# swesterfeld/audiowmark

Measured on AMD Instinct MI355X. Metric: audio seconds watermarked+decoded per wall-second (xRT), 44.1 kHz stereo, higher is better.
Workload: dtype f32; 1 GPU; 60 min stereo 44.1 kHz white noise per GPU resident in HBM, add+get incl. payload decode, payload 0123456789abcdef0011223344556677, strength 10; parallelism=1 GPU, patterns=108, payload_matches=104, ranks_seen=1

## Files before the change

### audiowmark_amd/csrc/hip/kernels.hip

```cpp
#include "kernels.hh"
#include "awm_fft.hip.h"
#include <cstdlib>
#include <algorithm>
#include <type_traits>
#include <atomic>

namespace awmk {

constexpr int NB = 81;
constexpr int MIN_BAND = 20;
constexpr int WAVES = 4;

typedef const int __attribute__ ((address_space (4))) *const_int_ptr;

__device__ __forceinline__ void
load_shared_tables (const DevTables& t, float2 *s_tw, float *s_win, float2 *s_twb)
{
  fft512_load_twiddles (t.tw512, s_tw);
  for (int i = threadIdx.x; i < 1024; i += blockDim.x)
    s_win[i] = t.window[i];
  if (s_twb)
    for (int i = threadIdx.x; i < NB; i += blockDim.x)
      s_twb[i] = t.tw1024[MIN_BAND + i];
}


__device__ __forceinline__ void
fetch_stereo (const float *pcm, long long idx, int avail, int lane, float (&l)[16], float (&r)[16])
{
  const float *p = pcm + idx * 2;
  if (avail >= 1024 && ((reinterpret_cast<uintptr_t> (p) & 15) == 0))
    {
      const float4 *p4 = reinterpret_cast<const float4 *> (p);
#pragma unroll
      for (int j = 0; j < 8; j++)
        {
          const float4 v = p4[lane + 64 * j];
          l[2 * j] = v.x; r[2 * j] = v.y; l[2 * j + 1] = v.z; r[2 * j + 1] = v.w;
        }
    }
  else if (avail >= 1024)
    {
      const float2 *p2 = reinterpret_cast<const float2 *> (p);
#pragma unroll
      for (int j = 0; j < 8; j++)
        {
          const float2 a = p2[2 * (lane + 64 * j)], b = p2[2 * (lane + 64 * j) + 1];
          l[2 * j] = a.x; r[2 * j] = a.y; l[2 * j + 1] = b.x; r[2 * j + 1] = b.y;
        }
    }
  else
    {
#pragma unroll
      for (int j = 0; j < 8; j++)
        {
          const int x = 2 * (lane + 64 * j);
          l[2 * j]     = x < avail     ? p[2 * x]     : 0.f;
          r[2 * j]     = x < avail     ? p[2 * x + 1] : 0.f;
          l[2 * j + 1] = x + 1 < avail ? p[2 * x + 2] : 0.f;
          r[2 * j + 1] = x + 1 < avail ? p[2 * x + 3] : 0.f;
        }
    }
}

__device__ __forceinline__ void
fetch_channel (const float *pcm, long long idx, int avail, int C, int ch, int lane, float (&v)[16])
{
  const float *p = pcm + idx * C + ch;
  if (C == 1 && avail >= 1024 && ((reinterpret_cast<uintptr_t> (p) & 7) == 0))
    {
      const float2 *p2 = reinterpret_cast<const float2 *> (p);
#pragma unroll
      for (int j = 0; j < 8; j++)
        {
          const float2 a = p2[lane + 64 * j];
          v[2 * j] = a.x; v[2 * j + 1] = a.y;
        }
    }
  else
    {
#pragma unroll
      for (int j = 0; j < 8; j++)
        {
          const int x = 2 * (lane + 64 * j);
          v[2 * j]     = x < avail     ? p[(long long) x * C]       : 0.f;
          v[2 * j + 1] = x + 1 < avail ? p[(long long) (x + 1) * C] : 0.f;
        }
    }
}

__device__ __forceinline__ void
window_pack (const float (&v)[16], const float *s_win, int lane, float2 (&z)[8])
{
  const float2 *w2 = reinterpret_cast<const float2 *> (s_win);
#pragma unroll
  for (int j = 0; j < 8; j++)
    {
      const float2 w = lds_ld (&w2[lane + 64 * j]);
      z[j] = make_float2 (__fmul_rn (v[2 * j], w.x), __fmul_rn (v[2 * j + 1], w.y));
    }
}

__global__ void __launch_bounds__ (64 * WAVES)
stft_full_kernel (DevTables t, const float *pcm, int C, long long start_index, long long hop, long long frame_count, float2 *out)
{
  __shared__ float2 s_tw[512];
  __shared__ float  s_win[1024];
  __shared__ float2 s_x[WAVES][XBUF_ELEMS];
  load_shared_tables (t, s_tw, s_win, nullptr);
  __syncthreads();

  const int lane = threadIdx.x & 63, wave = threadIdx.x >> 6;
  const long long item = (long long) blockIdx.x * WAVES + wave;
  if (item >= frame_count * C)
    return;
  const long long f = item / C;
  const int ch = int (item % C);
  float2 *xbuf = s_x[wave];

  float v[16];
  fetch_channel (pcm, start_index + f * hop, 1024, C, ch, lane, v);
  float2 z[8];
  window_pack (v, s_win, lane, z);
  fft512_forward (z, xbuf, s_tw, lane);
#pragma unroll
  for (int kc = 0; kc < 8; kc++)
    xbuf[kc * 64 + lane] = z[kc];
  wave_sync();
  float2 *o = out + item * 513;
  for (int k = lane; k <= 512; k += 64)
    {
      const float2 zk = xbuf[zpos (k & 511)], zm = xbuf[zpos ((512 - k) & 511)];
      o[k] = real_split (zk, zm, t.tw1024[k]);
    }
}

hipError_t
launch_stft_full (hipStream_t st, const DevTables& t, const float *pcm, int n_channels,
                  long long start_index, long long hop, long long frame_count, float2 *out)
{
  const long long items = frame_count * n_channels;
  if (items <= 0)
    return hipSuccess;
  const unsigned grid = unsigned ((items + WAVES - 1) / WAVES);
  hipLaunchKernelGGL (stft_full_kernel, dim3 (grid), dim3 (64 * WAVES), 0, st, t, pcm, n_channels, start_index, hop, frame_count, out);
  return hipGetLastError();
}


__device__ __forceinline__ int
zdpos (int k)
{
  const int kc = k >> 6;
  return (kc < 2 ? kc : kc - 4) * 64 + ((k >> 3) & 7) + 8 * (k & 7);
}


__device__ __forceinline__ void
frame_forward (float2 (&z)[8], float2 *xbuf, const float2 *s_tw, int lane)
{
  fft512_forward (z, xbuf, s_tw, lane);
  xbuf[0 * 64 + lane] = z[0];
  xbuf[1 * 64 + lane] = z[1];
  xbuf[6 * 64 + lane] = z[6];
  xbuf[7 * 64 + lane] = z[7];
  wave_sync();
}

__device__ __forceinline__ void
frame_forward2 (float2 (&za)[8], float2 (&zb)[8], float2 *xbuf, const float2 *s_tw, int lane)
{
  fft512_forward2 (za, zb, xbuf, s_tw, lane);
  lds_st (&xbuf[0 * 64 + lane], za[0]);
  lds_st (&xbuf[1 * 64 + lane], za[1]);
  lds_st (&xbuf[6 * 64 + lane], za[6]);
  lds_st (&xbuf[7 * 64 + lane], za[7]);
  lds_st (&xbuf[2 * 64 + lane], zb[0]);
  lds_st (&xbuf[3 * 64 + lane], zb[1]);
  lds_st (&xbuf[4 * 64 + lane], zb[6]);
  lds_st (&xbuf[5 * 64 + lane], zb[7]);
  wave_sync_pinned();
}

__device__ __forceinline__ int
zposb (int k)
{
  const int p = zpos (k);
  return p < 128 ? p + 128 : p - 128;
}

template<bool PINNED = false> __device__ __forceinline__ void
halfspec_store (float2 *zd, int k, float2 D, float2 O)
{
  const float2 lo = make_float2 (D.x - O.y, D.y + O.x), hi = make_float2 (D.x + O.y, O.x - D.y);
  if constexpr (PINNED)
    {
      lds_st (&zd[zdpos (k)], lo);
      lds_st (&zd[zdpos (512 - k)], hi);
    }
  else
    {
      zd[zdpos (k)] = lo;
      zd[zdpos (512 - k)] = hi;
    }
}

__device__ __forceinline__ void
frame_inverse (float2 (&z)[8], float2 *xbuf, float2 *zd, const float2 *s_tw, const float2 *s_tw3, int lane)
{
  wave_sync();
  const float2 zero = make_float2 (0.f, 0.f);
  z[0] = zd[0 * 64 + lane];
  z[1] = zd[1 * 64 + lane];
  z[2] = zero; z[3] = zero; z[4] = zero; z[5] = zero;
  z[6] = zd[2 * 64 + lane];
  z[7] = zd[3 * 64 + lane];
  wave_sync();
  fft512_inverse (z, xbuf, s_tw, s_tw3, lane);
}

__device__ __forceinline__ void
frame_inverse2 (float2 (&za)[8], float2 (&zb)[8], const float2 (&Da)[2], const float2 (&Oa)[2], const float2 (&Db)[2], const float2 (&Ob)[2],
                float2 *xbuf, float2 *zd, const float2 *s_tw, const float2 *s_tw3, int lane)
{
  const float2 zero = make_float2 (0.f, 0.f);
  wave_sync_pinned();
#pragma unroll
  for (int pass = 0; pass < 2; pass++)
    {
      const int k = MIN_BAND + lane + 64 * pass;
      if (k <= 100)
        halfspec_store<true> (zd, k, Da[pass], Oa[pass]);
    }
  wave_sync_pinned();
  za[0] = lds_ld (&zd[0 * 64 + lane]);
  za[1] = lds_ld (&zd[1 * 64 + lane]);
  za[2] = zero; za[3] = zero; za[4] = zero; za[5] = zero;
  za[6] = lds_ld (&zd[2 * 64 + lane]);
  za[7] = lds_ld (&zd[3 * 64 + lane]);
  wave_sync_pinned();
#pragma unroll
  for (int pass = 0; pass < 2; pass++)
    {
      const int k = MIN_BAND + lane + 64 * pass;
      if (k <= 100)
        halfspec_store<true> (zd, k, Db[pass], Ob[pass]);
    }
  wave_sync_pinned();
  zb[0] = lds_ld (&zd[0 * 64 + lane]);
  zb[1] = lds_ld (&zd[1 * 64 + lane]);
  zb[2] = zero; zb[3] = zero; zb[4] = zero; zb[5] = zero;
  zb[6] = lds_ld (&zd[2 * 64 + lane]);
  zb[7] = lds_ld (&zd[3 * 64 + lane]);
  wave_sync_pinned();
  fft512_inverse2 (za, zb, xbuf, s_tw, s_tw3, lane);
}

__device__ __forceinline__ void
frame_delta (float2 (&z)[8], const int8_t *mod_row, float nd_up, float nd_down,
             float2 *xbuf, float2 *zd, const float2 *s_tw, const float2 *s_tw3, const float2 *s_twb, int lane)
{
  frame_forward (z, xbuf, s_tw, lane);
#pragma unroll
  for (int pass = 0; pass < 2; pass++)
    {
      const int k = MIN_BAND + lane + 64 * pass;
      if (k <= 100)
        {
          const float2 w = s_twb[k - MIN_BAND];
          const float2 X = real_split (xbuf[zpos (k)], xbuf[zpos (512 - k)], w);
          const int mod = mod_row[k - MIN_BAND];
          float2 D = make_float2 (0.f, 0.f);
          if (mod)
            {
              const float abs2 = X.x * X.x + X.y * X.y;
              if (abs2 > 1e-14f)
                {
                  const float s = __builtin_amdgcn_exp2f (__builtin_amdgcn_logf (abs2) * (0.5f * (mod == 1 ? nd_up : nd_down))) - 1.0f;
                  D = make_float2 (X.x * s, X.y * s);
                }
            }
          halfspec_store (zd, k, D, cmulc (D, w));
        }
    }
  frame_inverse (z, xbuf, zd, s_tw, s_tw3, lane);
}

__device__ __forceinline__ void
frame_delta2 (float2 (&za)[8], float2 (&zb)[8], const int8_t *mod_row, float nd_up, float nd_down,
              float2 *xbuf, float2 *zd, const float2 *s_tw, const float2 *s_tw3, const float2 *s_twb, int lane)
{
  frame_forward2 (za, zb, xbuf, s_tw, lane);
  float2 Da[2], Db[2], Oa[2], Ob[2];
#pragma unroll
  for (int pass = 0; pass < 2; pass++)
    {
      const int k = MIN_BAND + lane + 64 * pass;
      Da[pass] = Db[pass] = Oa[pass] = Ob[pass] = make_float2 (0.f, 0.f);
      if (k <= 100)
        {
          const float2 w = s_twb[k - MIN_BAND];
          const float2 Xa = real_split (lds_ld (&xbuf[zpos (k)]), lds_ld (&xbuf[zpos (512 - k)]), w);
          const float2 Xb = real_split (lds_ld (&xbuf[zposb (k)]), lds_ld (&xbuf[zposb (512 - k)]), w);
          const int mod = mod_row[k - MIN_BAND];
          if (mod)
            {
              const float e = 0.5f * (mod == 1 ? nd_up : nd_down);
              const float abs2a = Xa.x * Xa.x + Xa.y * Xa.y, abs2b = Xb.x * Xb.x + Xb.y * Xb.y;
              if (abs2a > 1e-14f)
                {
                  const float s = __builtin_amdgcn_exp2f (__builtin_amdgcn_logf (abs2a) * e) - 1.0f;
                  Da[pass] = make_float2 (Xa.x * s, Xa.y * s);
                }
              if (abs2b > 1e-14f)
                {
                  const float s = __builtin_amdgcn_exp2f (__builtin_amdgcn_logf (abs2b) * e) - 1.0f;
                  Db[pass] = make_float2 (Xb.x * s, Xb.y * s);
                }
            }
          Oa[pass] = cmulc (Da[pass], w);
          Ob[pass] = cmulc (Db[pass], w);
        }
    }
  frame_inverse2 (za, zb, Da, Oa, Db, Ob, xbuf, zd, s_tw, s_tw3, lane);
}

__device__ __forceinline__ float
wave_max (float v)
{
#pragma unroll
  for (int off = 32; off > 0; off >>= 1)
    v = fmaxf (v, __shfl_xor (v, off));
  return v;
}

struct FramePlace
{
  bool own, own_prev;
  int b0, bound, pb0, pbound;
};

__device__ __forceinline__ FramePlace
frame_place (long long gs_m, int BS, long long first_block, bool own, bool own_prev)
{
  FramePlace fp;
  fp.own = own;
  fp.own_prev = own_prev;
  const long long b0 = gs_m >= 0 ? gs_m / BS : 0;
  const long long gs_p = gs_m - 1024;
  const long long pb0 = gs_p >= 0 ? gs_p / BS : 0;
  fp.b0 = int (b0 - first_block);
  fp.bound = int (std::min<long long> ((b0 + 1) * BS - gs_m, 2048));
  fp.pb0 = int (pb0 - first_block);
  fp.pbound = int (std::min<long long> ((pb0 + 1) * BS - gs_p, 2048));
  return fp;
}

template<int CV> __device__ __forceinline__ void
overlap_add_mix (float (&o)[CV][16], const float2 (&d)[CV][8], const float (&in)[CV][16], float (&head2)[CV][2], float (&tail_s1)[CV][2],
                 const float (&tail_in)[CV][2], float2 w1_head, float2 w2_head, float2 w1_tail, float2 w0_tail)
{
#pragma unroll
  for (int c = 0; c < CV; c++)
    {
      const float s1x = __fadd_rn (head2[c][0], __fmul_rn (d[c][0].x, w1_head.x));
      const float s1y = __fadd_rn (head2[c][1], __fmul_rn (d[c][0].y, w1_head.y));
      o[c][0] = __fadd_rn (s1x, in[c][0]);
      o[c][1] = __fadd_rn (s1y, in[c][1]);
      head2[c][0] = __fmul_rn (d[c][0].x, w2_head.x);
      head2[c][1] = __fmul_rn (d[c][0].y, w2_head.y);
#pragma unroll
      for (int j = 1; j < 7; j++)
        {
          o[c][2 * j]     = __fadd_rn (d[c][j].x, in[c][2 * j]);
          o[c][2 * j + 1] = __fadd_rn (d[c][j].y, in[c][2 * j + 1]);
        }
      o[c][14] = __fadd_rn (__fadd_rn (tail_s1[c][0], __fmul_rn (d[c][7].x, w0_tail.x)), tail_in[c][0]);
      o[c][15] = __fadd_rn (__fadd_rn (tail_s1[c][1], __fmul_rn (d[c][7].y, w0_tail.y)), tail_in[c][1]);
      tail_s1[c][0] = __fmul_rn (d[c][7].x, w1_tail.x);
      tail_s1[c][1] = __fmul_rn (d[c][7].y, w1_tail.y);
    }
}

template<int CV, bool RANGE> __device__ __forceinline__ void
emit_frame (float *out, unsigned int *block_max, const float (&o)[CV][16], long long m, const FramePlace& fp,
            long long n_frames, long long n_blocks, int C, int ch0, int lane)
{
  float max0 = 0.f, max1 = 0.f, pmax0 = 0.f, pmax1 = 0.f;
  const bool whole_m = (m + 1) * 1024 <= n_frames;
  if (fp.own && whole_m && fp.bound >= 1024)
    {
      const long long base = m * 1024;
#pragma unroll
      for (int j = 0; j < 7; j++)
        {
          const long long ls = base + 2 * (lane + 64 * j);
          if (CV == 2)
            *reinterpret_cast<float4 *> (out + ls * 2) = make_float4 (o[0][2 * j], o[CV - 1][2 * j], o[0][2 * j + 1], o[CV - 1][2 * j + 1]);
          else
            {
              float *p = out + ls * C + ch0;
              p[0] = o[0][2 * j];
// ... 1283 lines not shown
  const bool stereo = a.n_channels == 2 && stereo_aligned;
  const bool stage = stereo && lds_floats > 0 && span <= 4096 && (long long) RS_TILE * a.step + a.np < (1LL << 31);
  const int in_span = stage ? int (span) : 0;
  const size_t lds_bytes = size_t ((lds_floats + 1) & ~1) * sizeof (float) + size_t (in_span) * sizeof (float2);
  if (one && stereo)
    hipLaunchKernelGGL (resample_slice_kernel<2>, grid, dim3 (256), lds_bytes, st, a, *one, lds_floats, in_span, tiles_per_wg);
  else if (one)
    hipLaunchKernelGGL (resample_slice_kernel<0>, grid, dim3 (256), lds_bytes, st, a, *one, lds_floats, in_span, tiles_per_wg);
  else if (stereo)
    hipLaunchKernelGGL ((resample_slices_kernel<2, In>), grid, dim3 (256), lds_bytes, st, a, slices_dev, lds_floats, in_span, tiles_per_wg);
  else
    hipLaunchKernelGGL ((resample_slices_kernel<0, In>), grid, dim3 (256), lds_bytes, st, a, slices_dev, lds_floats, in_span, tiles_per_wg);
  return hipGetLastError();
}
hipError_t
launch_resample_slices (hipStream_t st, const ResampleArgs& a, const ResampleSlice *slices_dev, int n_slices, long long max_n_out, bool stereo_aligned)
{
  return launch_resample_slices_any (st, a, slices_dev, nullptr, n_slices, max_n_out, stereo_aligned);
}
hipError_t
launch_resample_slices_s16 (hipStream_t st, const ResampleArgs& a, const ResampleSlice *slices_dev, int n_slices, long long max_n_out, bool stereo_aligned)
{
  return launch_resample_slices_any<PcmS16> (st, a, slices_dev, nullptr, n_slices, max_n_out, stereo_aligned);
}
hipError_t
launch_resample_slice (hipStream_t st, const ResampleArgs& a, const ResampleSlice& slice)
{
  if (slice.n_in < 0 || slice.in0 < 0 || slice.out0 < 0)
    return hipErrorInvalidValue;
  const bool aligned = (reinterpret_cast<uintptr_t> (slice.in) & 7) == 0 && (reinterpret_cast<uintptr_t> (slice.out) & 7) == 0;
  return launch_resample_slices_any (st, a, nullptr, &slice, 1, slice.n_out, aligned);
}

bool
resample_span_takes_phase (const ResampleArgs& a, const ResampleSlice& s)
{
  const bool aligned = (reinterpret_cast<uintptr_t> (s.in) & 7) == 0 && (reinterpret_cast<uintptr_t> (s.out) & 7) == 0;
  const bool ratio = (a.np == 147 && a.step == 160 && a.hl == 18) || (a.np == 160 && a.step == 147 && a.hl == 16);
  return g_resample_phase && a.n_channels == 2 && aligned && ratio && s.out0 >= 0 && s.out0 % a.np == 0;
}
hipError_t
launch_resample_span (hipStream_t st, ResampleArgs a, ResampleSlice s)
{
  if (s.n_out <= 0)
    return hipSuccess;
  if (!resample_span_takes_phase (a, s))
    return launch_resample_slice (st, a, s);
  if (a.np == 147)
    return launch_resample_phase_span<147, 160, 18> (st, a, s);
  return launch_resample_phase_span<160, 147, 16> (st, a, s);
}

constexpr int MIX_RUN = 2048;

__global__ void __launch_bounds__ (256)
power_sums_kernel (const float *orig, const float *mixed, long long n_values, double *acc)
{
  __shared__ double s_d[4], s_s[4];
  double d2 = 0, s2 = 0;
  for (long long i = (long long) blockIdx.x * 256 + threadIdx.x; i < n_values; i += (long long) gridDim.x * 256)
    {
      const double o = orig[i], d = double (mixed[i]) - o;
      d2 += d * d;
      s2 += o * o;
    }
#pragma unroll
  for (int off = 32; off > 0; off >>= 1)
    {
      d2 += __shfl_xor (d2, off);
      s2 += __shfl_xor (s2, off);
    }
  if ((threadIdx.x & 63) == 0)
    {
      s_d[threadIdx.x >> 6] = d2;
      s_s[threadIdx.x >> 6] = s2;
    }
  __syncthreads();
  if (threadIdx.x == 0)
    {
      atomicAdd (acc, s_d[0] + s_d[1] + s_d[2] + s_d[3]);
      atomicAdd (acc + 1, s_s[0] + s_s[1] + s_s[2] + s_s[3]);
    }
}

hipError_t
launch_power_sums (hipStream_t st, const float *orig, const float *mixed, long long n_values, double *acc)
{
  if (n_values <= 0)
    return hipSuccess;
  const long long blocks = (n_values + 256 * 16 - 1) / (256 * 16);
  hipLaunchKernelGGL (power_sums_kernel, dim3 (unsigned (blocks < 4096 ? blocks : 4096)), dim3 (256), 0, st, orig, mixed, n_values, acc);
  return hipGetLastError();
}

__global__ void __launch_bounds__ (256)
mix_max_kernel (const float *orig, const float *wm, float *out, long long n_values, int C, unsigned int *block_max, long long n_blocks, int BS)
{
  __shared__ float s_m0[4], s_m1[4];
  const long long base = (long long) blockIdx.x * MIX_RUN;
  const long long f0 = base / C;
  const long long b0 = f0 / BS;
  const long long bound = (b0 + 1) * BS * C;
  float m0 = 0.f, m1 = 0.f;
  for (int j = 0; j < MIX_RUN / 256; j++)
    {
      const long long v = base + threadIdx.x + 256LL * j;
      if (v < n_values)
        {
          const float r = __fadd_rn (wm[v], orig[v]);
          out[v] = r;
          if (v < bound)
            m0 = fmaxf (m0, fabsf (r));
          else
            m1 = fmaxf (m1, fabsf (r));
        }
    }
  m0 = wave_max (m0);
  m1 = wave_max (m1);
  if ((threadIdx.x & 63) == 0)
    {
      s_m0[threadIdx.x >> 6] = m0;
      s_m1[threadIdx.x >> 6] = m1;
    }
  __syncthreads();
  if (threadIdx.x == 0 && block_max)
    {
      m0 = fmaxf (fmaxf (s_m0[0], s_m0[1]), fmaxf (s_m0[2], s_m0[3]));
      m1 = fmaxf (fmaxf (s_m1[0], s_m1[1]), fmaxf (s_m1[2], s_m1[3]));
      if (b0 < n_blocks && m0 > 0.f) atomicMax (block_max + b0, __float_as_uint (m0));
      if (b0 + 1 < n_blocks && m1 > 0.f) atomicMax (block_max + b0 + 1, __float_as_uint (m1));
    }
}

hipError_t
launch_mix_max (hipStream_t st, const float *orig, const float *wm, float *out, long long n_frames, int n_channels,
                unsigned int *block_max, long long n_blocks, int limiter_block)
{
  const long long n_values = n_frames * n_channels;
  if (n_values <= 0)
    return hipSuccess;
  if ((long long) limiter_block * n_channels < MIX_RUN)
    return hipErrorInvalidValue;
  hipLaunchKernelGGL (mix_max_kernel, dim3 (unsigned ((n_values + MIX_RUN - 1) / MIX_RUN)), dim3 (256), 0, st, orig, wm, out, n_values,
                      n_channels, block_max, n_blocks, limiter_block);
  return hipGetLastError();
}

template<class In = PcmF32, bool STORE = true> __device__ __forceinline__ void
mix_max_segment_body (const MixSegment& s, int C, int BS)
{
  __shared__ float s_m0[4], s_m1[4];
  const long long n_values = (s.pre + s.n_frames) * C, pre_values = s.pre * C;
  const long long base = (long long) blockIdx.x * MIX_RUN;
  if (base >= n_values)
    return;
  const long long start = s.first_sample - s.pre;
  const long long b0 = (start + base / C) / BS;
  const long long bound = ((b0 + 1) * BS - start) * C;
  const typename In::value *orig = reinterpret_cast<const typename In::value *> (s.orig);
  float m0 = 0.f, m1 = 0.f;
  for (int j = 0; j < MIX_RUN / 256; j++)
    {
      const long long v = base + threadIdx.x + 256LL * j;
      if (v < n_values)
        {
          float r = s.wm[v];
          if (v >= pre_values)
            {
              r = __fadd_rn (r, In::conv (orig[v - pre_values]));
              if (STORE)
                s.out[v - pre_values] = r;
            }
          if (v < bound)
            m0 = fmaxf (m0, fabsf (r));
          else
            m1 = fmaxf (m1, fabsf (r));
        }
    }
  m0 = wave_max (m0);
  m1 = wave_max (m1);
  if ((threadIdx.x & 63) == 0)
    {
      s_m0[threadIdx.x >> 6] = m0;
      s_m1[threadIdx.x >> 6] = m1;
    }
  __syncthreads();
  if (threadIdx.x == 0 && s.block_max)
    {
      m0 = fmaxf (fmaxf (s_m0[0], s_m0[1]), fmaxf (s_m0[2], s_m0[3]));
      m1 = fmaxf (fmaxf (s_m1[0], s_m1[1]), fmaxf (s_m1[2], s_m1[3]));
      const long long i0 = b0 - s.first_block, i1 = i0 + 1;
      if (i0 >= 0 && i0 < s.n_blocks && m0 > 0.f) atomicMax (s.block_max + i0, __float_as_uint (m0));
      if (i1 >= 0 && i1 < s.n_blocks && m1 > 0.f) atomicMax (s.block_max + i1, __float_as_uint (m1));
    }
}
__global__ void __launch_bounds__ (256)
mix_max_segments_kernel (const MixSegment *segs, int C, int BS)
{
  const MixSegment s = segs[blockIdx.y];
  mix_max_segment_body (s, C, BS);
}
__global__ void __launch_bounds__ (256)
mix_max_segment_kernel (MixSegment s, int C, int BS)
{
  mix_max_segment_body (s, C, BS);
}
__global__ void __launch_bounds__ (256)
max_segments_s16_kernel (const MixSegment *segs, int C, int BS)
{
  const MixSegment s = segs[blockIdx.y];
  mix_max_segment_body<PcmS16, false> (s, C, BS);
}

hipError_t
launch_mix_max_segments (hipStream_t st, const MixSegment *segs_dev, int n_segs, long long max_frames, int n_channels, int limiter_block)
{
  if (n_segs <= 0 || max_frames <= 0)
    return hipSuccess;
  if (n_segs > 65535 || n_channels < 1 || (long long) limiter_block * n_channels < MIX_RUN)
    return hipErrorInvalidValue;
  const long long max_values = max_frames * n_channels;
  hipLaunchKernelGGL (mix_max_segments_kernel, dim3 (unsigned ((max_values + MIX_RUN - 1) / MIX_RUN), unsigned (n_segs)), dim3 (256), 0, st,
                      segs_dev, n_channels, limiter_block);
  return hipGetLastError();
}
hipError_t
launch_max_segments_s16 (hipStream_t st, const MixSegment *segs_dev, int n_segs, long long max_frames, int n_channels, int limiter_block)
{
  if (n_segs <= 0 || max_frames <= 0)
    return hipSuccess;
  if (n_segs > 65535 || n_channels < 1 || (long long) limiter_block * n_channels < MIX_RUN)
    return hipErrorInvalidValue;
  const long long max_values = max_frames * n_channels;
  hipLaunchKernelGGL (max_segments_s16_kernel, dim3 (unsigned ((max_values + MIX_RUN - 1) / MIX_RUN), unsigned (n_segs)), dim3 (256), 0, st,
                      segs_dev, n_channels, limiter_block);
  return hipGetLastError();
}
hipError_t
launch_mix_max_segment (hipStream_t st, const MixSegment& seg, int n_channels, int limiter_block)
{
  const long long n_values = (seg.pre + seg.n_frames) * n_channels;
  if (n_values <= 0)
    return hipSuccess;
  if (n_channels < 1 || seg.pre < 0 || seg.first_sample < seg.pre || (long long) limiter_block * n_channels < MIX_RUN)
    return hipErrorInvalidValue;
  hipLaunchKernelGGL (mix_max_segment_kernel, dim3 (unsigned ((n_values + MIX_RUN - 1) / MIX_RUN)), dim3 (256), 0, st, seg, n_channels, limiter_block);
  return hipGetLastError();
}

__global__ void
fill_u32_kernel (unsigned int *p, unsigned int v, size_t n)
{
  const size_t i = (size_t) blockIdx.x * blockDim.x + threadIdx.x;
  if (i < n)
    p[i] = v;
}
hipError_t
launch_fill_u32 (hipStream_t st, unsigned int *p, unsigned int v, size_t n)
{
  if (!n)
    return hipSuccess;
  hipLaunchKernelGGL (fill_u32_kernel, dim3 (unsigned ((n + 255) / 256)), dim3 (256), 0, st, p, v, n);
  return hipGetLastError();
}


__device__ __forceinline__ long long
sync_stream_base (const SyncDbArgs& a, long long stream)
{
  if (a.stream_base)
    return a.stream_base[stream];
  if (a.streams_per_slice > 0)
    return a.base0 + (stream % a.streams_per_slice) * a.base_stride + (stream / a.streams_per_slice) * a.slice_stride;
  return a.base0 + stream * a.base_stride;
}

__device__ __forceinline__ void
sync_stream_range (const SyncDbArgs& a, long long stream, long long& first, long long& last)
{
  first = a.first;
  last = a.last;
  if (a.stream_range)
    {
      const long long g = stream / a.range_div;
      const long long slice = a.range_index ? a.range_index[g] : g;
      first = a.stream_range[2 * slice];
      last = a.stream_range[2 * slice + 1];
      if (first < 0)
        first = last = 0x7fffffffffffffffLL;
    }
}


template<int CV, bool SPLIT, int TLD> __global__ void __launch_bounds__ (64 * WAVES)
sync_db_kernel (DevTables t, SyncDbArgs a)
{
  constexpr int TILE_LD = TLD, TILE_MAX = TLD - 1, SPLIT_COLS = TILE_MAX / 2;
  __shared__ float2 s_tw[512];
  __shared__ float  s_win[1024];
  __shared__ float2 s_twb[NB];
  __shared__ float2 s_x[WAVES][XBUF_ELEMS];
  __shared__ float  s_tile[NB * TILE_LD];
  __shared__ char   s_have[TILE_MAX];
  const int lane = threadIdx.x & 63, wave = threadIdx.x >> 6;
  if (a.silent_frames_are_zero && a.skip_unread_silent_tiles)
    {
      long long stream = blockIdx.y, tile_idx = blockIdx.x;
      if (a.xcd_interleave)
        {
          const long long j = blockIdx.x >> 3;
          stream = j % a.n_streams;
          tile_idx = (j / a.n_streams) * 8 + (blockIdx.x & 7);
        }
      const long long base = sync_stream_base (a, stream);
      const int count = a.stream_count ? a.stream_count[stream] : a.count0;
      long long sil_first, sil_last;
      sync_stream_range (a, stream, sil_first, sil_last);
      const long long tile0 = tile_idx * a.tile_frames;
      if (tile0 >= count)
        return;
      const long long n_here = (count - tile0) < a.tile_frames ? count - tile0 : a.tile_frames;
      const long long idx_before = base + (tile0 - 2) * a.hop, idx_after = base + (tile0 + n_here + 1) * a.hop;
      const int C = a.n_channels;
      if ((idx_after + 1024) * C < sil_first || idx_before * C > sil_last)
        return;
    }
  load_shared_tables (t, s_tw, s_win, s_twb);
  __syncthreads();

  long long stream = blockIdx.y, tile_idx = blockIdx.x;
  if (a.xcd_interleave)
    {
      const long long j = blockIdx.x >> 3;
      stream = j % a.n_streams;
      tile_idx = (j / a.n_streams) * 8 + (blockIdx.x & 7);
    }
  const int plane_ch = blockIdx.z;
  const long long base = sync_stream_base (a, stream);
  const int count = a.stream_count ? a.stream_count[stream] : a.count0;
  long long sil_first, sil_last;
  sync_stream_range (a, stream, sil_first, sil_last);
  const int TF = a.tile_frames;
  const long long tile0 = tile_idx * TF;
  if (tile0 >= count)
    return;
  const int C = a.n_channels;
  float2 *xbuf = s_x[wave];
  const int n_here = (count - tile0) < TF ? int (count - tile0) : TF;

  for (int ff = wave; ff < n_here; ff += WAVES)
    {
      const long long idx = base + (tile0 + ff) * a.hop;
      const long long f_first = idx * C, f_last = (idx + 1024) * C;
      const bool outside = idx < 0 || idx + 1024 > a.n_frames;
      const bool skip = (f_last < sil_first) || (f_first > sil_last) || outside;
      float acc0 = 0.f, acc1 = 0.f;
      float split0 = 0.f, split1 = 0.f;
      if (!skip)
        {
          if (CV == 2)
            {
              float in[2][16];
              fetch_stereo (a.pcm, idx, 1024, lane, in[0], in[1]);
              float2 za[8], zb[8];
              window_pack (in[0], s_win, lane, za);
              window_pack (in[1], s_win, lane, zb);
              fft512_forward2 (za, zb, xbuf, s_tw, lane);
              const int k0 = MIN_BAND + lane, k1 = MIN_BAND + 64 + lane;
              const bool second = lane < NB - 64;
              float2 pa[4], pb[4];
              lds_st (&xbuf[0 * 64 + lane], za[0]);
              lds_st (&xbuf[1 * 64 + lane], za[1]);
              lds_st (&xbuf[6 * 64 + lane], za[6]);
              lds_st (&xbuf[7 * 64 + lane], za[7]);
              wave_sync();
              pa[0] = lds_ld (&xbuf[zpos (k0)]);
              pa[1] = lds_ld (&xbuf[zpos (512 - k0)]);
              pa[2] = lds_ld (&xbuf[zpos (second ? k1 : k0)]);
              pa[3] = lds_ld (&xbuf[zpos (512 - (second ? k1 : k0))]);
              wave_sync();
              lds_st (&xbuf[0 * 64 + lane], zb[0]);
              lds_st (&xbuf[1 * 64 + lane], zb[1]);
              lds_st (&xbuf[6 * 64 + lane], zb[6]);
              lds_st (&xbuf[7 * 64 + lane], zb[7]);
              wave_sync();
              pb[0] = lds_ld (&xbuf[zpos (k0)]);
              pb[1] = lds_ld (&xbuf[zpos (512 - k0)]);
              pb[2] = lds_ld (&xbuf[zpos (second ? k1 : k0)]);
              pb[3] = lds_ld (&xbuf[zpos (512 - (second ? k1 : k0))]);
              wave_sync();
              const float2 w0 = s_twb[lane], w1 = s_twb[second ? 64 + lane : lane];
              acc0 = __fadd_rn (acc0, db_from_complex (real_split (pa[0], pa[1], w0)));
              if (second)
                acc1 = __fadd_rn (acc1, db_from_complex (real_split (pa[2], pa[3], w1)));
              if (SPLIT)
                {
                  split0 = acc0;
                  split1 = acc1;
                  acc0 = acc1 = 0.f;
                }
              acc0 = __fadd_rn (acc0, db_from_complex (real_split (pb[0], pb[1], w0)));
              if (second)
                acc1 = __fadd_rn (acc1, db_from_complex (real_split (pb[2], pb[3], w1)));
            }
          else
            {
              const int c_begin = a.per_channel ? plane_ch : 0, c_end = a.per_channel ? plane_ch + 1 : C;
              for (int c = c_begin; c < c_end; c++)
                {
                  float in[16];
                  fetch_channel (a.pcm, idx, 1024, C, c, lane, in);
                  float2 z[8];
                  window_pack (in, s_win, lane, z);
                  fft512_forward (z, xbuf, s_tw, lane);
                  xbuf[0 * 64 + lane] = z[0];
                  xbuf[1 * 64 + lane] = z[1];
                  xbuf[6 * 64 + lane] = z[6];
                  xbuf[7 * 64 + lane] = z[7];
                  wave_sync();
                  {
                    const int k = MIN_BAND + lane;
                    acc0 = __fadd_rn (acc0, db_from_complex (real_split (xbuf[zpos (k)], xbuf[zpos (512 - k)], s_twb[lane])));
                  }
                  if (lane < NB - 64)
                    {
                      const int k = MIN_BAND + 64 + lane;
                      acc1 = __fadd_rn (acc1, db_from_complex (real_split (xbuf[zpos (k)], xbuf[zpos (512 - k)], s_twb[64 + lane])));
                    }
                  wave_sync();
                }
            }
        }
      else if (a.silent_frames_are_zero && !outside)
        {
          const float zero_db = db_from_complex (make_float2 (0.f, 0.f));
          const int n_ch = CV == 2 ? 2 : (a.per_channel ? 1 : C);
          for (int c = 0; c < n_ch; c++)
            {
              if (SPLIT && c == 1)
                {
                  split0 = acc0;
                  split1 = acc1;
                  acc0 = acc1 = 0.f;
                }
              acc0 = __fadd_rn (acc0, zero_db);
              acc1 = __fadd_rn (acc1, zero_db);
            }
        }
      if (SPLIT)
        {
          s_tile[lane * TILE_LD + ff] = split0;
          s_tile[lane * TILE_LD + SPLIT_COLS + ff] = acc0;
          if (lane < NB - 64)
            {
              s_tile[(64 + lane) * TILE_LD + ff] = split1;
              s_tile[(64 + lane) * TILE_LD + SPLIT_COLS + ff] = acc1;
            }
        }
      else
        {
          s_tile[lane * TILE_LD + ff] = acc0;
          if (lane < NB - 64)
            s_tile[(64 + lane) * TILE_LD + ff] = acc1;
        }
      if (lane == 0)
        s_have[ff] = skip ? 0 : 1;
    }
  __syncthreads();
  if (SPLIT)
    {
      for (int p = 0; p < 2; p++)
        {
          float *out = a.out + stream * a.out_stream_stride + (long long) p * NB * a.ld + tile0;
          for (int i = threadIdx.x; i < NB * n_here; i += blockDim.x)
            {
              const int band = i / n_here, ff = i - band * n_here;
              out[band * a.ld + ff] = s_tile[band * TILE_LD + p * SPLIT_COLS + ff];
            }
        }
    }
  else
    {
      const long long plane = a.per_channel ? plane_ch : 0;
      float *out = a.out + stream * a.out_stream_stride + plane * NB * a.ld + tile0;
      for (int i = threadIdx.x; i < NB * n_here; i += blockDim.x)
        {
          const int band = i / n_here, ff = i - band * n_here;
          out[band * a.ld + ff] = s_tile[band * TILE_LD + ff];
        }
    }
  if (a.have && plane_ch == 0)
    for (int i = threadIdx.x; i < n_here; i += blockDim.x)
      a.have[stream * a.have_stream_stride + tile0 + i] = s_have[i];
}

hipError_t
launch_sync_db (hipStream_t st, const DevTables& t, const SyncDbArgs& a)
{
  if (a.n_streams <= 0 || a.tile_frames <= 0 || a.tile_frames > 72)
    return a.n_streams <= 0 ? hipSuccess : hipErrorInvalidValue;
  int max_count = a.count0;
  if (max_count <= 0)
    return hipSuccess;
  const unsigned tiles = unsigned ((max_count + a.tile_frames - 1) / a.tile_frames);
  if (a.n_streams > 65535LL * 1)
    {
      SyncDbArgs b = a;
      long long done = 0;
      while (done < a.n_streams)
        {
          const long long n = (a.n_streams - done) > 65535 ? 65535 : (a.n_streams - done);
          b.n_streams = n;
          b.base0 = a.base0 + done * a.base_stride;
          b.stream_base = a.stream_base ? a.stream_base + done : nullptr;
          b.stream_count = a.stream_count ? a.stream_count + done : nullptr;
          b.out = a.out + done * a.out_stream_stride;
          b.have = a.have ? a.have + done * a.have_stream_stride : nullptr;
          hipError_t e = launch_sync_db (st, t, b);
          if (e != hipSuccess)
            return e;
          done += n;
        }
      return hipSuccess;
    }
  const bool small = a.tile_frames <= 32;
  if (a.n_channels == 2 && a.per_channel)
    {
      SyncDbArgs b = a;
      b.tile_frames = 16;
      const unsigned split_tiles = unsigned ((max_count + b.tile_frames - 1) / b.tile_frames);
      hipLaunchKernelGGL ((sync_db_kernel<2, true, 33>), dim3 (split_tiles, unsigned (a.n_streams), 1), dim3 (64 * WAVES), 0, st, t, b);
      return hipGetLastError();
    }
  const unsigned planes = a.per_channel ? unsigned (a.n_channels) : 1u;
  dim3 grid (tiles, unsigned (a.n_streams), planes);
  SyncDbArgs b = a;
  if (!a.stream_base && !a.stream_count && a.n_streams >= 2 && a.n_streams <= 8 && planes == 1)
    {
      b.xcd_interleave = 1;
      grid = dim3 (unsigned (((tiles + 7) / 8) * 8 * a.n_streams), 1, 1);
    }
  if (a.n_channels == 2 && !a.per_channel)
    {
      if (small)
        hipLaunchKernelGGL ((sync_db_kernel<2, false, 33>), grid, dim3 (64 * WAVES), 0, st, t, b);
      else
        hipLaunchKernelGGL ((sync_db_kernel<2, false, 73>), grid, dim3 (64 * WAVES), 0, st, t, b);
    }
  else
    {
      if (small)
        hipLaunchKernelGGL ((sync_db_kernel<1, false, 33>), grid, dim3 (64 * WAVES), 0, st, t, b);
      else
        hipLaunchKernelGGL ((sync_db_kernel<1, false, 73>), grid, dim3 (64 * WAVES), 0, st, t, b);
    }
  return hipGetLastError();
}

constexpr int SL_TILE = 16;

__device__ __forceinline__ double
dpp_from_lower_lane (double v)
{
  const int lo = __builtin_amdgcn_update_dpp (0, __double2loint (v), 0x138, 0xf, 0xf, true);
  const int hi = __builtin_amdgcn_update_dpp (0, __double2hiint (v), 0x138, 0xf, 0xf, true);
  return __hiloint2double (hi, lo);
}
__device__ __forceinline__ double
dpp_from_upper_lane (double v)
{
  const int lo = __builtin_amdgcn_update_dpp (0, __double2loint (v), 0x130, 0xf, 0xf, true);
  const int hi = __builtin_amdgcn_update_dpp (0, __double2hiint (v), 0x130, 0xf, 0xf, true);
  return __hiloint2double (hi, lo);
}

__device__ __forceinline__ long long
wave_uniform (long long v)
{
  const int lo = __builtin_amdgcn_readfirstlane (int (v)), hi = __builtin_amdgcn_readfirstlane (int (v >> 32));
  return (long long) (((unsigned long long) (unsigned int) hi << 32) | (unsigned int) lo);
}

typedef __attribute__ ((address_space (1))) float global_float;
__device__ __forceinline__ global_float *
uniform_global (const float *p)
{
  return (global_float *) (unsigned long long) wave_uniform ((long long) (unsigned long long) p);
}

template<int CV> __global__ void __launch_bounds__ (64 * WAVES) __attribute__ ((amdgpu_waves_per_eu (3, 3)))
sync_db_sliding_kernel (DevTables t, SyncDbArgs a)
{
  constexpr int SCRATCH_FLOATS = XBUF_ELEMS * 4 > NB * SL_TILE ? XBUF_ELEMS * 4 : NB * SL_TILE;
  __shared__ __attribute__ ((aligned (16))) float s_scratch[WAVES][SCRATCH_FLOATS];
  __shared__ unsigned char s_pos[WAVES][NB + 3];
  __shared__ __attribute__ ((aligned (16))) double s_delta[WAVES][SL_TILE * 8 * CV];
  __shared__ int s_nzd[WAVES][SL_TILE * CV];
  __shared__ int s_x0[WAVES][SL_TILE * CV];
  {
    const int w = threadIdx.x >> 6, l = threadIdx.x & 63;
    const long long s = (long long) blockIdx.x * WAVES + w;
    const long long tslice = (a.tables_per_slice && s < a.n_streams) ? (a.range_index ? a.range_index[s / a.range_div] : s / a.range_div) : 0;
    for (int b = l; b < NB; b += 64)
      s_pos[w][b] = (a.band_pos && s < a.n_streams) ? a.band_pos[(tslice * a.rows_per_plane + s % a.rows_per_plane) * NB + b] : (unsigned char) b;
  }
  __syncthreads();

  const int lane = threadIdx.x & 63, wave = threadIdx.x >> 6;
  const long long stream = (long long) blockIdx.x * WAVES + wave;
  if (stream >= a.n_streams)
    return;
  const long long perm_slice = a.tables_per_slice ? (a.range_index ? a.range_index[stream / a.range_div] : stream / a.range_div) : 0;
  const long long out_slot = wave_uniform (a.row_perm ? (stream / a.rows_per_plane) * a.rows_per_plane
                                                        + a.row_perm[perm_slice * a.rows_per_plane + stream % a.rows_per_plane] : stream);
  const long long base = wave_uniform (sync_stream_base (a, stream));
  const int count = __builtin_amdgcn_readfirstlane (a.stream_count ? a.stream_count[stream] : a.count0);
  if (count <= 0)
    return;
  long long sil_first, sil_last;
  sync_stream_range (a, stream, sil_first, sil_last);
  sil_first = wave_uniform (sil_first);
  sil_last = wave_uniform (sil_last);
  if (a.have && ((base + 8LL * (count - 1) + 1024) * CV < sil_first || base * CV > sil_last))
    {
      if (lane < count)
        a.have[out_slot * a.have_stream_stride + lane] = 0;
      if (lane == 0 && count > 64)
        a.have[out_slot * a.have_stream_stride + 64] = 0;
      return;
    }
  double2 *xbuf = reinterpret_cast<double2 *> (s_scratch[wave]);
  float *tile = s_scratch[wave];
  const int C = CV;
  const bool bins = lane < 42;
  const int kA = 19 + 2 * (bins ? lane : 0);

  double2 R[CV][2];
  int nz[CV];
  {
#pragma unroll
    for (int c = 0; c < CV; c++)
      {
        float in[16];
        fetch_channel (a.pcm, base, 1024, CV, c, lane, in);
        int cnt = 0;
#pragma unroll
        for (int j = 0; j < 16; j++)
          cnt += in[j] != 0.f;
        for (int o = 32; o > 0; o >>= 1)
          cnt += __shfl_xor (cnt, o);
        nz[c] = __builtin_amdgcn_readfirstlane (cnt);
        double2 z[8];
#pragma unroll
        for (int j = 0; j < 8; j++)
          z[j] = make_double2 (double (in[2 * j]), double (in[2 * j + 1]));
        fft512_forward_d (z, xbuf, t.tw512d, lane);
        xbuf[0 * 64 + lane] = z[0];
        xbuf[1 * 64 + lane] = z[1];
        xbuf[6 * 64 + lane] = z[6];
        xbuf[7 * 64 + lane] = z[7];
        wave_sync();
#pragma unroll
        for (int b = 0; b < 2; b++)
          {
            const int k = kA + b;
            R[c][b] = real_split_d (xbuf[zpos (k)], xbuf[zpos (512 - k)], t.slide[(k - 19) * 9 + 1]);
          }
        wave_sync();
      }
  }
  double2 tw[2][8];
  int k_tab = kA - 19;
  asm volatile ("" : "+v" (k_tab));
#pragma unroll
  for (int b = 0; b < 2; b++)
#pragma unroll
    for (int j = 0; j < 8; j++)
      tw[b][j] = t.slide[(k_tab + b) * 9 + j + 1];

  constexpr int FPL = 2 * CV;
  float f_in[FPL], f_out[FPL];
  auto fetch_block = [&] (int q) {
    const long long s0 = base + 128LL * q;
#pragma unroll
    for (int i = 0; i < FPL; i++)
      {
        const int e = lane * FPL + i;
        const int trans = SL_TILE * q + e / (8 * C);
        const bool need = trans + 1 < count;
        f_in[i] = need ? a.pcm[(s0 + 1024) * C + e] : 0.f;
        f_out[i] = trans < count ? a.pcm[s0 * C + e] : 0.f;
      }
  };
  auto publish_block = [&] () {
#pragma unroll
    for (int i = 0; i < FPL; i++)
      s_delta[wave][lane * FPL + i] = double (f_in[i]) - double (f_out[i]);
#pragma unroll
    for (int c = 0; c < CV; c++)
      {
        int dn = (f_in[c] != 0.f) - (f_out[c] != 0.f) + (f_in[CV + c] != 0.f) - (f_out[CV + c] != 0.f);
        dn += __shfl_xor (dn, 1);
        dn += __shfl_xor (dn, 2);
        if ((lane & 3) == 0)
          {
            s_nzd[wave][(lane >> 2) * CV + c] = dn;
            s_x0[wave][(lane >> 2) * CV + c] = f_out[c] != 0.f;
          }
      }
  };
  fetch_block (0);
  unsigned long long have_mask = 0;
  bool have_64 = false;

  for (int step = 0; step < count; step++)
    {
      if (step % SL_TILE == 0)
        {
          publish_block();
          wave_sync();
          fetch_block (step / SL_TILE + 1);
        }
      const long long idx = base + 8LL * step;
      const long long f_first = idx * C, f_last = (idx + 1024) * C;
      const bool skip = (f_last < sil_first) || (f_first > sil_last);
      float dbA = 0.f, dbB = 0.f;
      if (!skip)
        {
          if (step < 64)
            have_mask |= 1ULL << step;
          else
            have_64 = true;
#pragma unroll
          for (int c = 0; c < CV; c++)
            {
              if (nz[c] - __builtin_amdgcn_readfirstlane (s_x0[wave][(step % SL_TILE) * CV + c]) == 0)
                {
                  dbA = __fadd_rn (dbA, -96.f);
                  dbB = __fadd_rn (dbB, -96.f);
                  continue;
                }
              const double2 up = make_double2 (dpp_from_lower_lane (R[c][1].x), dpp_from_lower_lane (R[c][1].y));
              const double2 dn = make_double2 (dpp_from_upper_lane (R[c][0].x), dpp_from_upper_lane (R[c][0].y));
              const float xa_re = float (fma (2.0, R[c][0].x, -(up.x + R[c][1].x))) * 0x1p-10f;
              const float xa_im = float (fma (2.0, R[c][0].y, -(up.y + R[c][1].y))) * 0x1p-10f;
              const float xb_re = float (fma (2.0, R[c][1].x, -(R[c][0].x + dn.x))) * 0x1p-10f;
              const float xb_im = float (fma (2.0, R[c][1].y, -(R[c][0].y + dn.y))) * 0x1p-10f;
              dbA = __fadd_rn (dbA, db_from_complex (make_float2 (xa_re, xa_im)));
              dbB = __fadd_rn (dbB, db_from_complex (make_float2 (xb_re, xb_im)));
            }
        }
      const int col = step % SL_TILE;
      if (bins)
        {
          const int bandA = kA - MIN_BAND, bandB = bandA + 1;
          if (bandA >= 0 && bandA < NB)
            tile[col * NB + bandA] = dbA;
          if (bandB < NB)
            tile[col * NB + bandB] = dbB;
        }
      if (col == SL_TILE - 1 || step == count - 1)
        {
          wave_sync();
          const int t0 = step - col, n_cols = col + 1;
          float *out = a.out + out_slot * a.out_stream_stride + t0;
          for (int i = lane; i < NB * SL_TILE; i += 64)
            {
              const int band = i / SL_TILE, cc = i % SL_TILE;
              const int row = s_pos[wave][band];
              if (cc < n_cols && row != 255)
                out[row * a.ld + cc] = tile[cc * NB + band];
            }
          wave_sync();
        }
      if (step + 1 < count)
        {
          const double *dl = s_delta[wave] + (step % SL_TILE) * 8 * C;
#pragma unroll
          for (int c = 0; c < CV; c++)
            {
              double2 acc[2] = { R[c][0], R[c][1] };
#pragma unroll
              for (int j = 0; j < 8; j++)
                {
                  const double d = dl[j * C + c];
#pragma unroll
                  for (int b = 0; b < 2; b++)
                    {
                      if (j == 0)
                        acc[b].x = acc[b].x + d;
                      else
                        {
                          acc[b].x = fma (d, tw[b][j - 1].x, acc[b].x);
                          acc[b].y = fma (d, tw[b][j - 1].y, acc[b].y);
                        }
                    }
                }
#pragma unroll
              for (int b = 0; b < 2; b++)
                {
                  const double2 r = tw[b][7];
                  R[c][b] = make_double2 (acc[b].x * r.x - acc[b].y * r.y, acc[b].x * r.y + acc[b].y * r.x);
                }
              nz[c] += __builtin_amdgcn_readfirstlane (s_nzd[wave][(step % SL_TILE) * CV + c]);
              if (nz[c] == 0)
                R[c][0] = R[c][1] = make_double2 (0.0, 0.0);
            }
        }
      if (step % SL_TILE == SL_TILE - 1)
        wave_sync();
    }
  if (a.have && lane < count)
    a.have[out_slot * a.have_stream_stride + lane] = (have_mask >> lane) & 1;
  if (a.have && lane == 0 && count > 64)
    a.have[out_slot * a.have_stream_stride + 64] = have_64;
}

__global__ void __launch_bounds__ (64 * WAVES) __attribute__ ((amdgpu_waves_per_eu (3, 3)))
sync_db_sliding3_kernel (DevTables t, SyncDbArgs a)
{
  constexpr int CV = 2, LPC = 28;
  constexpr int TILE_FLOATS = 2 * NB * SL_TILE;
  constexpr int SCRATCH_FLOATS = XBUF_ELEMS * 4 > TILE_FLOATS ? XBUF_ELEMS * 4 : TILE_FLOATS;
  __shared__ __attribute__ ((aligned (16))) float s_scratch[WAVES][SCRATCH_FLOATS];
  __shared__ unsigned char s_pos[WAVES][NB + 3];
  __shared__ __attribute__ ((aligned (16))) double s_delta[WAVES][SL_TILE * 8 * CV];
  __shared__ int s_nzd[WAVES][SL_TILE * CV];
  __shared__ int s_x0[WAVES][SL_TILE * CV];
  {
    const int w = threadIdx.x >> 6, l = threadIdx.x & 63;
    const long long s = (long long) blockIdx.x * WAVES + w;
    const long long tslice = (a.tables_per_slice && s < a.n_streams) ? (a.range_index ? a.range_index[s / a.range_div] : s / a.range_div) : 0;
    for (int b = l; b < NB; b += 64)
      s_pos[w][b] = (a.band_pos && s < a.n_streams) ? a.band_pos[(tslice * a.rows_per_plane + s % a.rows_per_plane) * NB + b] : (unsigned char) b;
  }
  __syncthreads();

  const int lane = threadIdx.x & 63, wave = threadIdx.x >> 6;
  const long long stream = (long long) blockIdx.x * WAVES + wave;
  if (stream >= a.n_streams)
    return;
  const long long perm_slice = a.tables_per_slice ? (a.range_index ? a.range_index[stream / a.range_div] : stream / a.range_div) : 0;
  const long long out_slot = wave_uniform (a.row_perm ? (stream / a.rows_per_plane) * a.rows_per_plane
// ... 1991 lines not shown
```

Measured before the change: 759,800 xRT.

## Rework sync_db kernel bin extraction with cross-lane exchange and vectorized tile stores

The stereo sync spectrum kernel now takes its mirrored FFT bins through ds_bpermute cross-lane exchanges, using a lane-to-bin mapping, in place of four LDS store/load round trips with wave syncs per channel. The window is loaded once into registers and applied to both channels together. The aligned/unaligned PCM fetch paths merge into one 8-byte-aligned vector load. Full tiles are written out as float4 quads, and the per-element div/mod in the output loop is replaced by incremental indexing. Other changes: the silent-tile early exit is folded into the main index computation, xcd-interleave math moves to 32-bit with a power-of-two fast path, and overflow guards are added. The new lane-to-band mapping and bin ownership logic carry correctness risk.

Result: no change. 755,600 xRT, median of 2 (-0.6%).

```diff
diff --git a/audiowmark_amd/csrc/hip/kernels.hip b/audiowmark_amd/csrc/hip/kernels.hip
--- a/audiowmark_amd/csrc/hip/kernels.hip
+++ b/audiowmark_amd/csrc/hip/kernels.hip
@@ -29,24 +29,15 @@
 fetch_stereo (const float *pcm, long long idx, int avail, int lane, float (&l)[16], float (&r)[16])
 {
   const float *p = pcm + idx * 2;
-  if (avail >= 1024 && ((reinterpret_cast<uintptr_t> (p) & 15) == 0))
-    {
-      const float4 *p4 = reinterpret_cast<const float4 *> (p);
+  if (avail >= 1024)
+    {
+      typedef float pcm_quad __attribute__ ((ext_vector_type (4), aligned (8)));
+      const pcm_quad *p4 = reinterpret_cast<const pcm_quad *> (p);
 #pragma unroll
       for (int j = 0; j < 8; j++)
         {
-          const float4 v = p4[lane + 64 * j];
+          const pcm_quad v = p4[lane + 64 * j];
           l[2 * j] = v.x; r[2 * j] = v.y; l[2 * j + 1] = v.z; r[2 * j + 1] = v.w;
-        }
-    }
-  else if (avail >= 1024)
-    {
-      const float2 *p2 = reinterpret_cast<const float2 *> (p);
-#pragma unroll
-      for (int j = 0; j < 8; j++)
-        {
-          const float2 a = p2[2 * (lane + 64 * j)], b = p2[2 * (lane + 64 * j) + 1];
-          l[2 * j] = a.x; r[2 * j] = a.y; l[2 * j + 1] = b.x; r[2 * j + 1] = b.y;
         }
     }
   else
@@ -98,6 +89,26 @@
     {
       const float2 w = lds_ld (&w2[lane + 64 * j]);
       z[j] = make_float2 (__fmul_rn (v[2 * j], w.x), __fmul_rn (v[2 * j + 1], w.y));
+    }
+}
+
+__device__ __forceinline__ void
+window_load (const float *s_win, int lane, float2 (&w)[8])
+{
+  const float2 *w2 = reinterpret_cast<const float2 *> (s_win);
+#pragma unroll
+  for (int j = 0; j < 8; j++)
+    w[j] = lds_ld (&w2[lane + 64 * j]);
+}
+
+__device__ __forceinline__ void
+window_pack2 (const float (&va)[16], const float (&vb)[16], const float2 (&w)[8], float2 (&za)[8], float2 (&zb)[8])
+{
+#pragma unroll
+  for (int j = 0; j < 8; j++)
+    {
+      za[j] = make_float2 (__fmul_rn (va[2 * j], w[j].x), __fmul_rn (va[2 * j + 1], w[j].y));
+      zb[j] = make_float2 (__fmul_rn (vb[2 * j], w[j].x), __fmul_rn (vb[2 * j + 1], w[j].y));
     }
 }
 
@@ -1987,39 +1998,26 @@
   __shared__ float2 s_x[WAVES][XBUF_ELEMS];
   __shared__ float  s_tile[NB * TILE_LD];
   __shared__ char   s_have[TILE_MAX];
-  const int lane = threadIdx.x & 63, wave = threadIdx.x >> 6;
-  if (a.silent_frames_are_zero && a.skip_unread_silent_tiles)
-    {
-      long long stream = blockIdx.y, tile_idx = blockIdx.x;
-      if (a.xcd_interleave)
-        {
-          const long long j = blockIdx.x >> 3;
-          stream = j % a.n_streams;
-          tile_idx = (j / a.n_streams) * 8 + (blockIdx.x & 7);
-        }
-      const long long base = sync_stream_base (a, stream);
-      const int count = a.stream_count ? a.stream_count[stream] : a.count0;
-      long long sil_first, sil_last;
-      sync_stream_range (a, stream, sil_first, sil_last);
-      const long long tile0 = tile_idx * a.tile_frames;
-      if (tile0 >= count)
-        return;
-      const long long n_here = (count - tile0) < a.tile_frames ? count - tile0 : a.tile_frames;
-      const long long idx_before = base + (tile0 - 2) * a.hop, idx_after = base + (tile0 + n_here + 1) * a.hop;
-      const int C = a.n_channels;
-      if ((idx_after + 1024) * C < sil_first || idx_before * C > sil_last)
-        return;
-    }
-  load_shared_tables (t, s_tw, s_win, s_twb);
-  __syncthreads();
-
-  long long stream = blockIdx.y, tile_idx = blockIdx.x;
+  const int lane = threadIdx.x & 63, wave = __builtin_amdgcn_readfirstlane (threadIdx.x >> 6);
+
+  unsigned stream_u = blockIdx.y, tile_u = blockIdx.x;
   if (a.xcd_interleave)
     {
-      const long long j = blockIdx.x >> 3;
-      stream = j % a.n_streams;
-      tile_idx = (j / a.n_streams) * 8 + (blockIdx.x & 7);
-    }
+      const unsigned j = blockIdx.x >> 3, n = unsigned (a.n_streams);
+      unsigned q;
+      if ((n & (n - 1)) == 0)
+        {
+          q = j >> __builtin_ctz (n);
+          stream_u = j & (n - 1);
+        }
+      else
+        {
+          q = j / n;
+          stream_u = j - q * n;
+        }
+      tile_u = q * 8 + (blockIdx.x & 7);
+    }
+  const long long stream = stream_u, tile_idx = tile_u;
   const int plane_ch = blockIdx.z;
   const long long base = sync_stream_base (a, stream);
   const int count = a.stream_count ? a.stream_count[stream] : a.count0;
@@ -2030,8 +2028,25 @@
   if (tile0 >= count)
     return;
   const int C = a.n_channels;
+  const int n_here = (count - tile0) < TF ? int (count - tile0) : TF;
+  if (a.silent_frames_are_zero && a.skip_unread_silent_tiles)
+    {
+      const long long idx_before = base + (tile0 - 2) * a.hop, idx_after = base + (tile0 + n_here + 1) * a.hop;
+      if ((idx_after + 1024) * C < sil_first || idx_before * C > sil_last)
+        return;
+    }
+  load_shared_tables (t, s_tw, s_win, s_twb);
+  __syncthreads();
   float2 *xbuf = s_x[wave];
-  const int n_here = (count - tile0) < TF ? int (count - tile0) : TF;
+  float2 win[8];
+  if (CV == 2)
+    window_load (s_win, lane, win);
+  const int bin_m = 8 * (lane & 7) + (lane >> 3);
+  const int band0 = CV == 2 ? bin_m - MIN_BAND : lane, band1 = CV == 2 ? 64 + bin_m - MIN_BAND : 64 + lane;
+  const bool own0 = CV == 2 ? bin_m >= MIN_BAND : true, own1 = band1 < NB;
+  const int mirror = (64 - bin_m) & 63;
+  const int xchg_addr = 4 * (((mirror >> 3) & 7) + 8 * (mirror & 7));
+  auto xchg = [xchg_addr] (float v) { return __int_as_float (__builtin_amdgcn_ds_bpermute (xchg_addr, __float_as_int (v))); };
 
   for (int ff = wave; ff < n_here; ff += WAVES)
     {
@@ -2048,45 +2063,26 @@
               float in[2][16];
               fetch_stereo (a.pcm, idx, 1024, lane, in[0], in[1]);
               float2 za[8], zb[8];
-              window_pack (in[0], s_win, lane, za);
-              window_pack (in[1], s_win, lane, zb);
+              window_pack2 (in[0], in[1], win, za, zb);
               fft512_forward2 (za, zb, xbuf, s_tw, lane);
-              const int k0 = MIN_BAND + lane, k1 = MIN_BAND + 64 + lane;
-              const bool second = lane < NB - 64;
-              float2 pa[4], pb[4];
-              lds_st (&xbuf[0 * 64 + lane], za[0]);
-              lds_st (&xbuf[1 * 64 + lane], za[1]);
-              lds_st (&xbuf[6 * 64 + lane], za[6]);
-              lds_st (&xbuf[7 * 64 + lane], za[7]);
-              wave_sync();
-              pa[0] = lds_ld (&xbuf[zpos (k0)]);
-              pa[1] = lds_ld (&xbuf[zpos (512 - k0)]);
-              pa[2] = lds_ld (&xbuf[zpos (second ? k1 : k0)]);
-              pa[3] = lds_ld (&xbuf[zpos (512 - (second ? k1 : k0))]);
-              wave_sync();
-              lds_st (&xbuf[0 * 64 + lane], zb[0]);
-              lds_st (&xbuf[1 * 64 + lane], zb[1]);
-              lds_st (&xbuf[6 * 64 + lane], zb[6]);
-              lds_st (&xbuf[7 * 64 + lane], zb[7]);
-              wave_sync();
-              pb[0] = lds_ld (&xbuf[zpos (k0)]);
-              pb[1] = lds_ld (&xbuf[zpos (512 - k0)]);
-              pb[2] = lds_ld (&xbuf[zpos (second ? k1 : k0)]);
-              pb[3] = lds_ld (&xbuf[zpos (512 - (second ? k1 : k0))]);
-              wave_sync();
-              const float2 w0 = s_twb[lane], w1 = s_twb[second ? 64 + lane : lane];
-              acc0 = __fadd_rn (acc0, db_from_complex (real_split (pa[0], pa[1], w0)));
-              if (second)
-                acc1 = __fadd_rn (acc1, db_from_complex (real_split (pa[2], pa[3], w1)));
+              float2 ma0 = make_float2 (xchg (za[7].x), xchg (za[7].y)), ma1 = make_float2 (xchg (za[6].x), xchg (za[6].y));
+              float2 mb0 = make_float2 (xchg (zb[7].x), xchg (zb[7].y)), mb1 = make_float2 (xchg (zb[6].x), xchg (zb[6].y));
+              if (lane == 0)
+                {
+                  ma1 = za[7];
+                  mb1 = zb[7];
+                }
+              const float2 w0 = s_twb[own0 ? band0 : 0], w1 = s_twb[own1 ? band1 : 0];
+              acc0 = __fadd_rn (acc0, db_from_complex (real_split (za[0], ma0, w0)));
+              acc1 = __fadd_rn (acc1, db_from_complex (real_split (za[1], ma1, w1)));
               if (SPLIT)
                 {
                   split0 = acc0;
                   split1 = acc1;
                   acc0 = acc1 = 0.f;
                 }
-              acc0 = __fadd_rn (acc0, db_from_complex (real_split (pb[0], pb[1], w0)));
-              if (second)
-                acc1 = __fadd_rn (acc1, db_from_complex (real_split (pb[2], pb[3], w1)));
+              acc0 = __fadd_rn (acc0, db_from_complex (real_split (zb[0], mb0, w0)));
+              acc1 = __fadd_rn (acc1, db_from_complex (real_split (zb[1], mb1, w1)));
             }
           else
             {
@@ -2134,44 +2130,87 @@
         }
       if (SPLIT)
         {
-          s_tile[lane * TILE_LD + ff] = split0;
-          s_tile[lane * TILE_LD + SPLIT_COLS + ff] = acc0;
-          if (lane < NB - 64)
-            {
-              s_tile[(64 + lane) * TILE_LD + ff] = split1;
-              s_tile[(64 + lane) * TILE_LD + SPLIT_COLS + ff] = acc1;
+          if (own0)
+            {
+              s_tile[band0 * TILE_LD + ff] = split0;
+              s_tile[band0 * TILE_LD + SPLIT_COLS + ff] = acc0;
+            }
+          if (own1)
+            {
+              s_tile[band1 * TILE_LD + ff] = split1;
+              s_tile[band1 * TILE_LD + SPLIT_COLS + ff] = acc1;
             }
         }
       else
         {
-          s_tile[lane * TILE_LD + ff] = acc0;
-          if (lane < NB - 64)
-            s_tile[(64 + lane) * TILE_LD + ff] = acc1;
+          if (own0)
+            s_tile[band0 * TILE_LD + ff] = acc0;
+          if (own1)
+            s_tile[band1 * TILE_LD + ff] = acc1;
         }
       if (lane == 0)
         s_have[ff] = skip ? 0 : 1;
     }
   __syncthreads();
-  if (SPLIT)
-    {
-      for (int p = 0; p < 2; p++)
-        {
-          float *out = a.out + stream * a.out_stream_stride + (long long) p * NB * a.ld + tile0;
-          for (int i = threadIdx.x; i < NB * n_here; i += blockDim.x)
-            {
-              const int band = i / n_here, ff = i - band * n_here;
+  constexpr int COLS = SPLIT ? SPLIT_COLS : TILE_MAX, PLANES = SPLIT ? 2 : 1, QUADS = COLS / 4;
+  static_assert (COLS % 4 == 0, "a full tile is written in quads");
+  const long long plane0 = SPLIT ? 0 : (a.per_channel ? plane_ch : 0);
+  float *out0 = a.out + stream * a.out_stream_stride + plane0 * NB * a.ld + tile0;
+  if (n_here == COLS)
+    {
+      constexpr int N_QUADS = NB * PLANES * QUADS, ROUNDS = (N_QUADS + 64 * WAVES - 1) / (64 * WAVES);
+      const bool wide = (reinterpret_cast<uintptr_t> (out0) & 15) == 0 && (a.ld & 3) == 0;
+      float v[ROUNDS][4];
+#pragma unroll
+      for (int r = 0; r < ROUNDS; r++)
+        {
+          const int i = threadIdx.x + r * 64 * WAVES;
+          if (ROUNDS * 64 * WAVES == N_QUADS || i < N_QUADS)
+            {
+              const int band = i / (PLANES * QUADS), q = i - band * (PLANES * QUADS);
+#pragma unroll
+              for (int e = 0; e < 4; e++)
+                v[r][e] = s_tile[band * TILE_LD + 4 * q + e];
+            }
+        }
+#pragma unroll
+      for (int r = 0; r < ROUNDS; r++)
+        {
+          const int i = threadIdx.x + r * 64 * WAVES;
+          if (ROUNDS * 64 * WAVES == N_QUADS || i < N_QUADS)
+            {
+              const int band = i / (PLANES * QUADS), q = i - band * (PLANES * QUADS);
+              const int p = q / QUADS, col = 4 * (q - p * QUADS);
+              float *o = out0 + ((long long) p * NB + band) * a.ld + col;
+              if (wide)
+                *reinterpret_cast<float4 *> (o) = make_float4 (v[r][0], v[r][1], v[r][2], v[r][3]);
+              else
+                {
+#pragma unroll
+                  for (int e = 0; e < 4; e++)
+                    o[e] = v[r][e];
+                }
+            }
+        }
+    }
+  else
+    {
+      const int step_band = (64 * WAVES) / n_here, step_ff = (64 * WAVES) - step_band * n_here;
+      for (int p = 0; p < PLANES; p++)
+        {
+          float *out = out0 + (long long) p * NB * a.ld;
+          int band = int (threadIdx.x) / n_here, ff = int (threadIdx.x) - band * n_here;
+          while (band < NB)
+            {
               out[band * a.ld + ff] = s_tile[band * TILE_LD + p * SPLIT_COLS + ff];
-            }
-        }
-    }
-  else
-    {
-      const long long plane = a.per_channel ? plane_ch : 0;
-      float *out = a.out + stream * a.out_stream_stride + plane * NB * a.ld + tile0;
-      for (int i = threadIdx.x; i < NB * n_here; i += blockDim.x)
-        {
-          const int band = i / n_here, ff = i - band * n_here;
-          out[band * a.ld + ff] = s_tile[band * TILE_LD + ff];
+              band += step_band;
+              ff += step_ff;
+              if (ff >= n_here)
+                {
+                  ff -= n_here;
+                  band++;
+                }
+            }
         }
     }
   if (a.have && plane_ch == 0)
@@ -2187,6 +2226,8 @@
   int max_count = a.count0;
   if (max_count <= 0)
     return hipSuccess;
+  if (max_count > 0x7fffffff - 72)
+    return hipErrorInvalidValue;
   const unsigned tiles = unsigned ((max_count + a.tile_frames - 1) / a.tile_frames);
   if (a.n_streams > 65535LL * 1)
     {
@@ -2220,10 +2261,11 @@
   const unsigned planes = a.per_channel ? unsigned (a.n_channels) : 1u;
   dim3 grid (tiles, unsigned (a.n_streams), planes);
   SyncDbArgs b = a;
-  if (!a.stream_base && !a.stream_count && a.n_streams >= 2 && a.n_streams <= 8 && planes == 1)
+  const long long interleaved = ((tiles + 7LL) / 8) * 8 * a.n_streams;
+  if (!a.stream_base && !a.stream_count && a.n_streams >= 2 && a.n_streams <= 8 && planes == 1 && interleaved <= 0x7fffffffLL)
     {
       b.xcd_interleave = 1;
-      grid = dim3 (unsigned (((tiles + 7) / 8) * 8 * a.n_streams), 1, 1);
+      grid = dim3 (unsigned (interleaved), 1, 1);
     }
   if (a.n_channels == 2 && !a.per_channel)
     {
```
